# gitouni/Spatial-Temporal-LiDAR-camera-Calibration

Measured on AMD Instinct MI355X. Metric: IBA residual+Jacobian evals/sec, higher is better.
Workload: dtype f64; 1 GPU; configs[1]-shaped synthetic street scene split over the GPUs: 200 keyframes x 10000 pts (2.0M pts), 2000 keypoints/KF, IBACalib cost (3d-2d + 3d-3d plane + hand-eye) + iba_local normal equations per candidate; frames_this_rank=200, points_per_frame=10000, keypoints_per_frame=2000, total_frames=200, total_points=2000000, plane_cache=1, parallelism=frames sharded over 1 GPU(s), 1 all-reduce of 4096 doubles per call, launch=single process, no collective, rccl_ranks=0

## Files before the change

include/iba_mi355x_debug.h:

```cpp
#ifndef IBA_MI355X_DEBUG_H
#define IBA_MI355X_DEBUG_H

#include "iba_mi355x.h"

#ifdef __cplusplus
extern "C" {
#endif

iba_status iba_last_kernel_ms(iba_handle* h, float* frame_kernel_ms, float* total_ms);
iba_status iba_set_timing(iba_handle* h, int32_t enable);
iba_status iba_last_phase_ms(iba_handle* h, float* assoc_kernel_ms, float* nn_kernel_ms, float* rest_ms);
iba_status iba_debug_phase_cycles(iba_handle* h, uint64_t out8[8], int32_t reset);
iba_status iba_debug_phase_cycles12(iba_handle* h, uint64_t out12[12], int32_t reset);
int32_t iba_debug_last_assoc2_threads(const iba_handle* h);
int32_t iba_debug_factor_ranges(const iba_handle* h, int32_t B);
iba_status iba_debug_last_partials(iba_handle* h, double* out, int32_t B);
int32_t iba_debug_last_path(const iba_handle* h);
iba_status iba_debug_plan_groups(const double* x, int32_t B, double max_fx, double max_px, int32_t max_groups, int32_t* group_of, double* group_px, int32_t* n_groups);
int32_t iba_debug_anchor_builds(const iba_handle* h);
int32_t iba_debug_pairs_builds(const iba_handle* h);
int32_t iba_debug_last_pairs_threads(const iba_handle* h);
int32_t iba_debug_pair_list(iba_handle* h, int32_t slot, int32_t frame, uint32_t* out_pairs, int32_t cap);
double iba_debug_nn_left_to_tree(iba_handle* h);
int32_t iba_debug_last_nn_threads(const iba_handle* h);
int32_t iba_debug_last_nn_list(const iba_handle* h);
double iba_debug_mean_pairs(iba_handle* h);
iba_status iba_debug_cand(const double x[7], double out58[58]);
int64_t iba_debug_rescans(iba_handle* h, int32_t reset);
iba_status iba_debug_counters(iba_handle* h, uint32_t out4[4], int32_t reset);
iba_status iba_debug_pair_lists(iba_handle* h, int32_t out3[3]);
iba_status iba_debug_nn(iba_handle* h, int32_t frame, const double* q_xyz, int32_t n, int32_t mode, uint32_t* out_idx, double* out_d2);
iba_status iba_debug_plane(iba_handle* h, int32_t frame, uint32_t point, int32_t which, double out5[5], int32_t* k);
iba_status iba_debug_scan_threads(iba_handle* h, int32_t threads);
int32_t iba_debug_last_scan_threads(const iba_handle* h);

iba_status iba_mads_selftest(int32_t problem, const double* x0, const iba_mads_options* opt, iba_mads_result* res);
iba_status iba_calibrate_mads_trace(iba_handle* h, const double* x0, const iba_mads_options* opt, iba_mads_result* res, double* trace, int32_t cap, int32_t* n_trace);
iba_status iba_calibrate_mads_record(iba_handle* h, const double* x0, const iba_mads_options* opt, iba_mads_result* res, double* trace, int32_t cap, int32_t* n_trace,
                                     int32_t* batch_sizes, int32_t cap_batches, int32_t* n_batches);
// ... 14 lines not shown
```

spatial-temporal-lidar-camera-calibration_amd/__init__.py:

```python
import ctypes as C
import os
import subprocess

import numpy as np

from .abi import (ICP_NMOM, SCAN_NMOM, IbaSubmapDesc, IbaScanEdge, IbaScanOptions, IbaScanResult, IbaIcpOptions, IbaIcpResult, IBA_MAX_BATCH, IbaCreateOptions, IbaLmOptions, IbaLmResult, IbaMadsOptions, IbaMadsResult, IbaBbo, IbaCostOut, IbaNormalOut, IbaParams, IbaProblemDesc, Problem, copy_params,
                  reference_yaml_params)

_HERE = os.path.dirname(os.path.abspath(__file__))
LIB_PATH = os.environ.get("IBA_LIB", os.path.join(_HERE, "libiba_mi355x.so"))
HEADER_PATH = os.path.join(os.path.dirname(_HERE), "include", "iba_mi355x.h")
HEADER_PATHS = [HEADER_PATH, os.path.join(os.path.dirname(_HERE), "include", "iba_mi355x_debug.h")]

STATUS = {0: "IBA_OK", 1: "IBA_ERR_INVALID_ARG", 2: "IBA_ERR_NO_DEVICE", 3: "IBA_ERR_HIP", 4: "IBA_ERR_UNSUPPORTED", 5: "IBA_ERR_STATE", 6: "IBA_ERR_IO"}


class IbaError(RuntimeError):
    def __init__(self, status, msg):
        super().__init__(f"{STATUS.get(status, status)}: {msg}")
        self.status = status


def build_extension(force=False):
    src_dir = os.path.join(_HERE, "csrc")
# ... 403 lines not shown
        self.lib.iba_debug_last_scan_threads.restype = C.c_int32
        return int(self.lib.iba_debug_last_scan_threads(self.h))

    def debug_factor_ranges(self, B):
        self.lib.iba_debug_factor_ranges.argtypes = [C.c_void_p, C.c_int32]
        self.lib.iba_debug_factor_ranges.restype = C.c_int32
        return int(self.lib.iba_debug_factor_ranges(self.h, C.c_int32(B)))

    @property
    def last_nn_threads(self):
        self.lib.iba_debug_last_nn_threads.argtypes = [C.c_void_p]
        self.lib.iba_debug_last_nn_threads.restype = C.c_int32
        return int(self.lib.iba_debug_last_nn_threads(self.h))

    @property
    def last_nn_list(self):
        self.lib.iba_debug_last_nn_list.argtypes = [C.c_void_p]
        self.lib.iba_debug_last_nn_list.restype = C.c_int32
        return int(self.lib.iba_debug_last_nn_list(self.h))

    def debug_last_partials(self, B):
        out = np.zeros((B, partial_stride()))
        self._chk(self.lib.iba_debug_last_partials(self.h, _p(out), C.c_int32(B)))
        return out

    def eval_full_partial(self, x, d_partials_ptr, stream_ptr=None):
        x = self._x(x)
        self._chk(self.lib.iba_eval_full_partial(self.h, _p(x), C.c_int32(len(x)), C.c_void_p(d_partials_ptr), C.c_void_p(stream_ptr)))

    @property
# ... 254 lines not shown
```

spatial-temporal-lidar-camera-calibration_amd/csrc/iba_capi.hip:

```cpp
#include <hip/hip_runtime.h>

#include <algorithm>
#include <atomic>
#include <cfloat>
#include <chrono>
#include <cmath>
#include <cstdio>
#include <cstring>
#include <limits>
#include <string>
#include <thread>
#include <vector>

#include "../../include/iba_mi355x.h"
#include "../../include/iba_mi355x_debug.h"
#include "iba_build.hpp"
#include "iba_host_math.hpp"
#include "iba_internal.hpp"
namespace iba {
const char* debug_env(const char* name) {
    const char* e = std::getenv("IBA_DEBUG_ENV");
    return (e && std::atoi(e) != 0) ? std::getenv(name) : nullptr;
}
}
// ... 58 lines not shown
    int factor_waves_forced = 0;
    F2Layout f2lay{};
    DevBuf<KpRec> d_kp_rec;
    DevBuf<ScanRec> d_scan_rec;
    bool scan_rec_valid = false;
    bool jets_fold = true;
    bool factor_rec = true;
    DevBuf<double> d_ffr;
    DevBuf<double2> d_kp_c;
    int nn_dbg = 0;
    bool nn_list = false;
    int nn_list_workers = 0;
    int n_cus = 256;
    int last_nn_threads = 0;
    int last_nn_list = 0;
    int nn_cg_max = kMaxGroup < 8 ? kMaxGroup : 8;
    int nn_small_min_b = 12;
    bool nn_small = false;
    bool nn_cg_fixed = false;
    bool nn_rounds = true;
    DevBuf<uint32_t> d_lcount, d_lcount_frozen;
    uint32_t max_slots = 0;
    uint32_t lstride = 1;
    int nn_ns = 1;
    DevBuf<double> d_nn_partials;
    hipEvent_t ev_mid = nullptr;
    float last_assoc_ms = 0.f, last_nn_ms = 0.f;
    LdsLayout alay2{};
    int assoc2_flreg_on = 1;
    DevBuf<PairRec> d_pairs;
// ... 203 lines not shown
}

bool layout_nn(const iba_handle* h, NNLayout& L, const int max_group = kMaxGroup) {
    L = NNLayout{};
    uint32_t off = 0;
    L.off_nodes = off; off += 8u * std::max(h->maxNodes, 1u);
    off = align_up(off, 16); L.off_misc = off; off += 128u;
    off = align_up(off, 16); L.off_cd = off; off += 8u * (uint32_t)kCdDoubles * (uint32_t)max_group;
    off = align_up(off, 16); L.off_res = off; off += 8u * kSliceW * (uint32_t)max_group;
    L.off_ovf = off; off += 4u * kSliceW * (uint32_t)max_group;
    L.total = off;
    off = align_up(off, 16); L.off_res2 = off;
    return L.total <= kLdsBytes;
}

int assoc2_q(const iba_handle* h, int threads = kThreads) { return !h->assoc2_flreg_on ? 0 : (h->maxKw <= 2u * (uint32_t)threads ? 2 : (h->maxKw <= 4u * (uint32_t)threads ? 4 : 0)); }
int assoc2_threads(const iba_handle* h, int blocks) {
    if (h->assoc2_threads_forced) return h->assoc2_threads_forced;
    if (blocks < h->assoc2_small_min_blocks) return kThreads;
    return assoc2_q(h, 256) != 0 || assoc2_q(h, kThreads) == 0 ? 256 : kThreads;
}
bool layout_assoc2(const iba_handle* h, LdsLayout& L) {
    const uint32_t rel_slots = std::max<uint32_t>(h->max_slots, 1u);
    const uint32_t red_bytes = 8u * kWaves * 4u + 8u * rel_slots * 12u + 4u * kWaves + 16u;
    L = LdsLayout{};
    L.rel_slots = rel_slots;
    uint32_t off = 0;
    const uint32_t Kp = (std::max(h->maxK, 1u) + 3u) & ~3u;
    L.off_best_d2 = off; off += 8u * Kp;
    L.off_best_idx = off; off += 4u * Kp;
// ... 467 lines not shown
    if (h->timing) HIP_TRY(h, hipEventRecord(h->ev_mid, st));
    if (refit && (want & 1)) {
        if (wide_fit) hipLaunchKernelGGL((iba_fit_kernel<4, 1>), fit_grid, dim3(64), 0, st, dp, h->dprm, fl, h->d_frefit.p, lc, (int)h->lstride, slot_base, want);
        else hipLaunchKernelGGL((iba_fit_kernel<2, 1>), fit_grid, dim3(64), 0, st, dp, h->dprm, fl, h->d_frefit.p, lc, (int)h->lstride, slot_base, want);
        HIP_TRY(h, hipGetLastError());
    }
    bool he_in_search = false;
    if (search) {
        const int he_blocks = (want & 2) ? (B * nf + nn_threads / 2 - 1) / (nn_threads / 2) : 0;
        he_in_search = he_blocks > 0;
        const dim3 grid(8 * per_xcd * ngroups * NS + ((he_blocks + 7) & ~7)), block(nn_threads);
        NNArgs na{dp, h->dprm, nl, (unsigned long long)(h->anchor_set_elems * sizeof(SetPt)), h->nn_rounds ? 1u : 0u, {0}};
        std::memcpy(na.anchor_sel, h->anchor_sel, sizeof(na.anchor_sel));
        const bool wA = (want & 1) != 0, wC = (want & 2) && h->dprm.use_3d3d;
        const SetPt* anchor = sets ? h->d_anchor.p : nullptr;
        auto launch_nn = [&](auto mode_tag) {
            constexpr int MODE = decltype(mode_tag)::value;
            h->last_nn_nrec = nn_nrec; h->last_nn_B = B;
            const int heb = MODE == kRefitSums ? 0 : he_blocks;
            const dim3 grid_m(MODE == kRefitSums ? 8 * per_xcd * ngroups * NS : grid.x);
            auto go = [&](auto kern) { hipLaunchKernelGGL(kern, grid_m, block, nl.total, st, na, dc, B, CG, NS, h->d_nn_partials.p, nn_nrec, fl, lc, (int)h->lstride, h->nn_dbg, h->d_frefit.p, anchor, h->d_he.p, heb); };
            h->last_nn_list = 0; h->last_nn_threads = nn_threads;
            const bool small_bufs = (size_t)B * nf * h->lstride * 16u < 0xFFFFFF00ull && (size_t)kAnchorSets * h->anchor_set_elems * sizeof(SetPt) < 0xFFFFFF00ull && (size_t)dp.n_kp_total * 16u < 0x80000000ull;
            int CGl = 1; { const int capl = B >= 12 ? 8 : (B >= 6 ? 4 : 2); while (CGl < std::min(B, capl)) CGl <<= 1; }
            if (sets && MODE == 0 && h->nn_list && small_bufs && CGl >= 4 && (kSliceW * (uint32_t)CGl) % (2u * (uint32_t)kNLThreads) == 0u && (kSliceW * (uint32_t)CGl) / (uint32_t)kNLThreads <= 4u) {
                NNLayout ll{};
                {
                    uint32_t off = 0;
                    ll.off_nodes = off; off += 8u * std::max(h->maxNodes, 1u);
                    off = align_up(off, 16); ll.off_misc = off; off += 128u;
                    off = align_up(off, 16); ll.off_cd = off; off += 8u * (uint32_t)kCdDoubles * (uint32_t)kNLMaxGroup;
                    off = align_up(off, 16); ll.off_res = off; off += 8u * kSliceW * (uint32_t)kNLMaxGroup;
                    ll.off_ovf = off; off += 4u * kSliceW * (uint32_t)kNLMaxGroup;
                    ll.total = off; off = align_up(off, 16); ll.off_res2 = off;
                }
                const uint32_t lds = align_up(ll.off_res2 + 8u * kSliceW * (uint32_t)kNLMaxGroup, 16);
                const int ngl = (B + CGl - 1) / CGl;
                const int hebl = (want & 2) ? (B * nf + kNLThreads / 2 - 1) / (kNLThreads / 2) : 0;
                const int per_cu = h->nn_list_workers > 0 ? h->nn_list_workers : std::max(1, std::min(4 * IBA_NN_LIST_WAVES * 64 / kNLThreads, (int)(kLdsBytes / lds)));
                const int R = std::max(1, std::min(per_xcd * NS, (h->n_cus * per_cu) / (8 * ngl)));
                h->last_nn_list = R;
                NNArgs nal = na; nal.lay = ll;
                const dim3 grid_l(8 * ngl * R + ((hebl + 7) & ~7));
                auto gol = [&](auto kern) { hipLaunchKernelGGL(kern, grid_l, dim3(kNLThreads), lds, st, nal, dc, B, CGl, NS, R, h->d_nn_partials.p, nn_nrec, fl, lc, (int)h->lstride, h->nn_dbg, anchor, h->d_he.p, hebl); };
                const bool four = (kSliceW * (uint32_t)CGl) / (uint32_t)kNLThreads == 4u;
                if (wA && wC) { if (four) gol(iba_nn_list_kernel<3, 4>); else gol(iba_nn_list_kernel<3, 2>); }
                else if (wA) { if (four) gol(iba_nn_list_kernel<1, 4>); else gol(iba_nn_list_kernel<1, 2>); }
                else { if (four) gol(iba_nn_list_kernel<2, 4>); else gol(iba_nn_list_kernel<2, 2>); }
            }
            else if (MODE == 0 && nn_small) {
                if (sets) { if (wA && wC) go(iba_nn_kernel<3, 0, 1, kNNThreadsSmall>); else if (wA) go(iba_nn_kernel<1, 0, 1, kNNThreadsSmall>); else go(iba_nn_kernel<2, 0, 1, kNNThreadsSmall>); }
                else { if (wA && wC) go(iba_nn_kernel<3, 0, 0, kNNThreadsSmall>); else if (wA) go(iba_nn_kernel<1, 0, 0, kNNThreadsSmall>); else go(iba_nn_kernel<2, 0, 0, kNNThreadsSmall>); }
            }
            else if (sets && MODE != kRefitSums) { if (wA && wC) go(iba_nn_kernel<3, MODE, 1>); else if (wA) go(iba_nn_kernel<1, MODE, 1>); else go(iba_nn_kernel<2, MODE, 1>); }
            else { if (wA && wC) go(iba_nn_kernel<3, MODE, 0>); else if (wA) go(iba_nn_kernel<1, MODE, 0>); else go(iba_nn_kernel<2, MODE, 0>); }
        };
        if (refit) launch_nn(std::integral_constant<int, kRefitSearch>{}); else launch_nn(std::integral_constant<int, 0>{});
        HIP_TRY(h, hipGetLastError());
        if (refit) {
            const int w2 = (wA ? 1 : 0) | (wC ? 2 : 0);
            if (wide_fit) hipLaunchKernelGGL((iba_fit_kernel<4, 2>), fit_grid, dim3(64), 0, st, dp, h->dprm, fl, h->d_frefit.p, lc, (int)h->lstride, slot_base, w2);
            else hipLaunchKernelGGL((iba_fit_kernel<2, 2>), fit_grid, dim3(64), 0, st, dp, h->dprm, fl, h->d_frefit.p, lc, (int)h->lstride, slot_base, w2);
            HIP_TRY(h, hipGetLastError());
// ... 314 lines not shown
    if (const char* e = dbg_env("IBA_ASSOC2_THREADS")) { const int v = std::atoi(e); h->assoc2_threads_forced = (v == 256 || v == kThreads) ? v : 0; }
    if (const char* e = dbg_env("IBA_ASSOC2_SMALL_MIN")) h->assoc2_small_min_blocks = std::max(0, std::atoi(e));
    if (const char* e = dbg_env("IBA_PAIR_GROUPS")) h->max_groups = std::max(1, std::min(kMaxPairGroups, std::atoi(e)));
    if (const char* e = dbg_env("IBA_CHAIN_FOLD")) h->chain_fold = std::atoi(e) != 0;
    if (const char* e = dbg_env("IBA_MAX_CHAIN")) h->chain_cap = std::atoi(e);
    h->chain_cap = std::max(1, std::min(h->chain_cap, (int)kMaxChain));
    if (!layout_assoc(h, h->alay)) { delete h; return fail(nullptr, IBA_ERR_UNSUPPORTED, "keypoints per frame exceed the LDS plan"); }
    if (!layout_assoc2(h, h->alay2) || 8u * (uint32_t)kPairStage + 160u + 2u * std::max(h->maxCoarse, 1u) + 8u * std::max(h->maxK, 1u) > kLdsBytes) h->common_mode = 0;
    if (dbg_env("IBA_LAYOUT_DEBUG")) std::fprintf(stderr, "[iba] assoc LDS: total %u B, queue %u entries, pairs %u, bitmap@%u; maxK %u maxKw %u\n", h->alay.total, h->alay.cand_cap, h->alay.pair_cap, h->alay.off_bitmap, h->maxK, h->maxKw);
    { NNLayout probe; if (!layout_nn(h, probe)) { delete h; return fail(nullptr, IBA_ERR_UNSUPPORTED, "kd tree exceeds the LDS plan of the search kernel"); } }
    h->lstride = std::max(1u, std::min(h->maxK, h->maxKw));
    h->nn_ns = (int)((h->lstride + kSliceW - 1u) / kSliceW) | 1;
    h->nn_small = 8u * std::max(h->maxNodes, 1u) <= 6144u;
    if (const char* e = dbg_env("IBA_NN_SMALL")) h->nn_small = std::atoi(e) != 0;
    if (const char* e = dbg_env("IBA_NN_SMALL_MIN_B")) h->nn_small_min_b = std::max(1, std::atoi(e));

    auto bail = [&](const char* what, hipError_t er) { std::string m = std::string(what) + ": " + hipGetErrorString(er); iba_destroy(h); return fail(nullptr, IBA_ERR_HIP, m); };
#define UP(buf, vec) do { hipError_t _e = h->buf.upload(vec); if (_e != hipSuccess) return bail("upload " #buf, _e); } while (0)
    {
        std::vector<float> frame_box(8 * (size_t)std::max(nf, 1), qnan);
        for (int lf = 0; lf < nf; ++lf) {
            float mn[3] = {INFINITY, INFINITY, INFINITY}, mx[3] = {-INFINITY, -INFINITY, -INFINITY};
            for (uint32_t c0 = 0; c0 < hdr[lf].P; c0 += (uint32_t)kChunk) {
                const float* bx = &chunk_box[8 * (size_t)(hdr[lf].box_base + c0 / (uint32_t)kChunk)];
                for (int a = 0; a < 3; ++a) { if (bx[a] < mn[a]) mn[a] = bx[a]; if (bx[4 + a] > mx[a]) mx[a] = bx[4 + a]; }
            }
            if (hdr[lf].P > 0) for (int a = 0; a < 3; ++a) { frame_box[8 * (size_t)lf + a] = mn[a]; frame_box[8 * (size_t)lf + 4 + a] = mx[a]; }
        }
        h->h_frame_box = frame_box;
        UP(d_frame_box, frame_box);
// ... 94 lines not shown
        const void* a2[12] = {(const void*)iba_assoc2_kernel<2, false, kThreads>, (const void*)iba_assoc2_kernel<2, true, kThreads>, (const void*)iba_assoc2_kernel<4, false, kThreads>, (const void*)iba_assoc2_kernel<4, true, kThreads>,
                              (const void*)iba_assoc2_kernel<0, false, kThreads>, (const void*)iba_assoc2_kernel<0, true, kThreads>,
                              (const void*)iba_assoc2_kernel<2, false, 256>, (const void*)iba_assoc2_kernel<2, true, 256>, (const void*)iba_assoc2_kernel<4, false, 256>, (const void*)iba_assoc2_kernel<4, true, 256>,
                              (const void*)iba_assoc2_kernel<0, false, 256>, (const void*)iba_assoc2_kernel<0, true, 256>};
        for (const void* fn : a2) if (h->common_mode > 0 && (er = hipFuncSetAttribute(fn, hipFuncAttributeMaxDynamicSharedMemorySize, (int)h->alay2.total)) != hipSuccess) return bail("hipFuncSetAttribute", er);
    }
    if ((er = hipFuncSetAttribute((const void*)iba_anchor_kernel, hipFuncAttributeMaxDynamicSharedMemorySize, (int)kLdsBytes)) != hipSuccess) return bail("hipFuncSetAttribute", er);
    const void* nfns[15] = {(const void*)iba_nn_kernel<1, 0, 0>, (const void*)iba_nn_kernel<2, 0, 0>, (const void*)iba_nn_kernel<3, 0, 0>, (const void*)iba_nn_kernel<1, 1, 0>, (const void*)iba_nn_kernel<2, 1, 0>,
                            (const void*)iba_nn_kernel<3, 1, 0>, (const void*)iba_nn_kernel<1, 2, 0>, (const void*)iba_nn_kernel<2, 2, 0>, (const void*)iba_nn_kernel<3, 2, 0>,
                            (const void*)iba_nn_kernel<1, 0, 1>, (const void*)iba_nn_kernel<2, 0, 1>, (const void*)iba_nn_kernel<3, 0, 1>, (const void*)iba_nn_kernel<1, 1, 1>, (const void*)iba_nn_kernel<2, 1, 1>,
                            (const void*)iba_nn_kernel<3, 1, 1>};
    for (const void* fn : nfns)
        if ((er = hipFuncSetAttribute(fn, hipFuncAttributeMaxDynamicSharedMemorySize, (int)kLdsBytes)) != hipSuccess) return bail("hipFuncSetAttribute", er);
    const void* sfns[6] = {(const void*)iba_nn_kernel<1, 0, 0, kNNThreadsSmall>, (const void*)iba_nn_kernel<2, 0, 0, kNNThreadsSmall>, (const void*)iba_nn_kernel<3, 0, 0, kNNThreadsSmall>,
                           (const void*)iba_nn_kernel<1, 0, 1, kNNThreadsSmall>, (const void*)iba_nn_kernel<2, 0, 1, kNNThreadsSmall>, (const void*)iba_nn_kernel<3, 0, 1, kNNThreadsSmall>};
    for (const void* fn : sfns)
        if ((er = hipFuncSetAttribute(fn, hipFuncAttributeMaxDynamicSharedMemorySize, (int)kLdsBytes)) != hipSuccess) return bail("hipFuncSetAttribute", er);
    const void* lfns[6] = {(const void*)iba_nn_list_kernel<1, 2>, (const void*)iba_nn_list_kernel<2, 2>, (const void*)iba_nn_list_kernel<3, 2>, (const void*)iba_nn_list_kernel<1, 4>, (const void*)iba_nn_list_kernel<2, 4>, (const void*)iba_nn_list_kernel<3, 4>};
    for (const void* fn : lfns)
        if ((er = hipFuncSetAttribute(fn, hipFuncAttributeMaxDynamicSharedMemorySize, (int)kLdsBytes)) != hipSuccess) return bail("hipFuncSetAttribute", er);

    {
        DevBuf<int32_t> okb; std::vector<int32_t> z(1, 0);
        er = okb.upload(z);
        if (er != hipSuccess) return bail("kernarg probe", er);
        hipLaunchKernelGGL(iba_kernarg_probe_kernel, dim3(1), dim3(1), 0, h->stream, KArgs{h->dev_problem(), h->dprm, h->alay}, okb.p);
        int32_t okv = 0;
        er = hipStreamSynchronize(h->stream);
        if (er == hipSuccess) er = hipMemcpy(&okv, okb.p, sizeof(okv), hipMemcpyDeviceToHost);
        okb.release();
// ... 209 lines not shown
iba_status iba_debug_phase_cycles(iba_handle* h, uint64_t out8[8], int32_t reset) {
    if (!h || !h->d_diag.p || !out8) return IBA_ERR_INVALID_ARG;
    if (hipSetDevice(h->device) != hipSuccess || hipStreamSynchronize(h->stream) != hipSuccess) return fail(h, IBA_ERR_HIP, "sync");
    if (hipMemcpy(out8, h->d_diag.p + 8, 64, hipMemcpyDeviceToHost) != hipSuccess) return fail(h, IBA_ERR_HIP, "copy");
    if (reset && hipMemset(h->d_diag.p + 8, 0, 64) != hipSuccess) return fail(h, IBA_ERR_HIP, "memset");
    return IBA_OK;
}
iba_status iba_debug_phase_cycles12(iba_handle* h, uint64_t out12[12], int32_t reset) {
    if (!h || !h->d_diag.p || !out12) return IBA_ERR_INVALID_ARG;
    if (hipSetDevice(h->device) != hipSuccess || hipStreamSynchronize(h->stream) != hipSuccess) return fail(h, IBA_ERR_HIP, "sync");
    if (hipMemcpy(out12, h->d_diag.p + 8, 96, hipMemcpyDeviceToHost) != hipSuccess) return fail(h, IBA_ERR_HIP, "copy");
    if (reset && hipMemset(h->d_diag.p + 8, 0, 96) != hipSuccess) return fail(h, IBA_ERR_HIP, "memset");
    return IBA_OK;
}
int32_t iba_debug_last_nn_threads(const iba_handle* h) { return h ? h->last_nn_threads : -1; }
int32_t iba_debug_last_nn_list(const iba_handle* h) { return h ? h->last_nn_list : -1; }
int32_t iba_debug_pairs_builds(const iba_handle* h) { return h ? h->pairs_builds : -1; }
int32_t iba_debug_last_pairs_threads(const iba_handle* h) { return h ? h->last_pairs_threads : -1; }
int32_t iba_debug_pair_list(iba_handle* h, int32_t slot, int32_t frame, uint32_t* out_pairs, int32_t cap) {
    if (h && slot < 0) slot = h->last_mean_pairs_slot;
    if (!h || slot < 0 || slot >= kMaxPairGroups || frame < 0 || frame >= h->n_frames || cap < 0 || (cap > 0 && !out_pairs)) return -1;
    if (!h->d_pairs.p || !h->d_pcounts.p || h->pair_cap <= 0) return 0;
    if (hipSetDevice(h->device) != hipSuccess || hipStreamSynchronize(h->stream) != hipSuccess) return -1;
    uint32_t c = 0;
    if (hipMemcpy(&c, h->d_pcounts.p + h->amap.cnt_off[slot] + (size_t)frame * kCountStride, sizeof(uint32_t), hipMemcpyDeviceToHost) != hipSuccess) return -1;
    const int32_t n = (int32_t)std::min<uint32_t>(c, (uint32_t)h->pair_cap);
    const int32_t m = std::min(n, cap);
    if (m > 0) {
        std::vector<PairRec> v((size_t)m);
        if (hipMemcpy(v.data(), h->d_pairs.p + ((size_t)slot * h->n_frames + (size_t)frame) * (size_t)h->pair_cap, (size_t)m * sizeof(PairRec), hipMemcpyDeviceToHost) != hipSuccess) return -1;
// ... 376 lines not shown
```

spatial-temporal-lidar-camera-calibration_amd/csrc/iba_split_kernels.hpp:

```cpp
#pragma once
#include "iba_kernels.hpp"
#include "iba_pair_plan.hpp"

namespace iba {

#ifndef IBA_PAIRS_CUT
#define IBA_PAIRS_CUT 0
#endif
#ifndef IBA_PAIRS_BLOCK_CUT
#define IBA_PAIRS_BLOCK_CUT 0
#endif
#ifndef IBA_NN_EXP
#define IBA_NN_EXP 0
#endif
#ifndef IBA_NN_THREADS
#define IBA_NN_THREADS 256
#endif
constexpr int kNNThreadsSmall = 64;
constexpr int kNNThreads = IBA_NN_THREADS;
constexpr int kNNWaves = kNNThreads / 64;
#ifndef IBA_NN_SLICE
#define IBA_NN_SLICE 128
#endif
constexpr uint32_t kSliceW = IBA_NN_SLICE;
// ... 5 lines not shown
    uint32_t off_nodes, off_res, off_misc, off_cd, off_ovf, total;
    uint32_t off_res2;
};
constexpr int kCdDoubles = 14;
#ifndef IBA_NN_WAVES
#define IBA_NN_WAVES 5
#endif
#ifndef IBA_NN_ROUND_LEAVES
#define IBA_NN_ROUND_LEAVES 8
#endif
#ifndef IBA_NN_LEAF_BATCH
#define IBA_NN_LEAF_BATCH 4
#endif
#ifndef IBA_NN_SETS_WAVES
#define IBA_NN_SETS_WAVES 4
#endif
constexpr int kAnchorSets = 2;
struct NNArgs {
    DevProblem dp; DevParams prm; NNLayout lay;
    unsigned long long anchor_set_bytes;
    uint32_t nn_rounds;
    uint8_t anchor_sel[kMaxChain];
};

constexpr uint32_t kFlagC = 1u;
constexpr int kRefitSearch = 1, kRefitSums = 2;
#ifdef IBA_DIAG_COUNTERS
#define IBA_DIAG_COUNT(cond, slot) do { if (cond) atomicAdd(dp.diag + (slot), 1u); } while (0)
#else
#define IBA_DIAG_COUNT(cond, slot) do { } while (0)
// ... 1831 lines not shown
                const PlaneRec rc = planes_cost[bp[i]];
                if (!(rc.far_d2 < prm.min_diff_dist2) && !(rc.k < prm.norm_min_pts) && !(rc.reg_sum / (double)(rc.k - 1) > prm.norm_reg_threshold)) { sp.flags |= 2u; sp.nx = rc.nx; sp.ny = rc.ny; sp.nz = rc.nz; }
            }
        }
        *(SetPt*)anchor_pt(row, (uint32_t)i) = sp;
        if (i == 0) hd.d1 = sqrt(bd[0]);
        if (i == 1) hd.da1_lo = sp.da_lo;
        hd.dM = sqrt(bd[i]);
        ++cnt;
    }
    hd.count = cnt;
    if (cnt < (uint32_t)kSetM) hd.dM = INFINITY;
    *(AnchorHdr*)row = hd;
}

template <int WHICH, int REFIT, int SETS, int T = kNNThreads>
__global__ __launch_bounds__(T) __attribute__((amdgpu_waves_per_eu(SETS ? IBA_NN_SETS_WAVES : IBA_NN_WAVES, SETS ? IBA_NN_SETS_WAVES : IBA_NN_WAVES))) void iba_nn_kernel(NNArgs ka_by_value, const Cand* __restrict__ cands, int B, int CG, int NS,
                                                                                                  double* __restrict__ nn_partials, int nn_nrec, uint4* __restrict__ flist,
                                                                                                  const uint32_t* __restrict__ lcount, int flist_stride, int dbg, double4* __restrict__ frefit,
                                                                                                  const SetPt* __restrict__ anchor, double* __restrict__ he_out, int he_blocks) {
    extern __shared__ __align__(16) unsigned char smem[];
    if ((int)blockIdx.x < he_blocks) {
        const int nfh = ka_by_value.dp.n_frames;
        const int i = (int)blockIdx.x * (T / 2) + (int)(threadIdx.x >> 1);
        const bool live = i < B * nfh;
        const int ii = live ? i : 0;
        const double v = he_term(ka_by_value.dp.frames[ii % nfh], cands[ii / nfh], threadIdx.x & 1, live);
        if (live && !(threadIdx.x & 1)) he_out[i] = v;
        return;
    }
    const uint32_t bid = blockIdx.x - (uint32_t)((he_blocks + 7) & ~7);
    constexpr int refit = REFIT;
    typedef __attribute__((address_space(4))) const NNArgs NNArgsC;
    NNArgsC* ka = (NNArgsC*)__builtin_amdgcn_kernarg_segment_ptr();
    (void)ka_by_value;
#define dp (ka->dp)
#define prm (ka->prm)
#define lay (ka->lay)
    constexpr int kMaxGroup = T / 32 < 16 ? T / 32 : 16, kCoopLimit = T / 2;
    static_assert((int)(kSliceW * (uint32_t)kMaxGroup) - kCoopLimit >= T / 2 * 4 && 4 * (2 * kMaxGroup + 4) <= 128, "LDS plan of the block shape");
    const int tid = threadIdx.x, lane = tid & 63;
#ifdef IBA_DIAG_COUNTERS
    unsigned long long nn_t[8] = {0, 0, 0, 0, 0, 0, 0, 0}, nn_last = __builtin_readcyclecounter();
#define NN_TICK(i) do { const unsigned long long _t = __builtin_readcyclecounter(); nn_t[i] += _t - nn_last; nn_last = _t; } while (0)
#else
#define NN_TICK(i) do { } while (0)
#endif
    const int nf = dp.n_frames;
    const int per_xcd = (nf + 7) / 8;
    const int NG = (B + CG - 1) / CG;
    const int per_frame = NG * NS;
    if (blockIdx.x < (uint32_t)((he_blocks + 7) & ~7)) return;
    const int xcd = bid & 7, jj = bid >> 3;
    const int f = xcd + 8 * (jj / per_frame);
    if (f >= nf || jj / per_frame >= per_xcd) return;
    const int g = (jj % per_frame) / NS, sl = (jj % per_frame) % NS;
    const FrameHdr& h = dp.frames[f];
    const uint32_t P = h.P, D = h.depth;
    const int cands_here = min(CG, B - g * CG);
    constexpr uint32_t kWantMask = ((WHICH & 2) ? kFlagC : 0u) | ((WHICH & 1) ? kFlagA : 0u);

    TreeNode* s_nodes = (TreeNode*)(smem + lay.off_nodes);
    double* s_res = (double*)(smem + lay.off_res);
    uint32_t* s_n = (uint32_t*)(smem + lay.off_misc);
    uint32_t* s_ctr = s_n + kMaxGroup;
    double* s_cd = (double*)(smem + lay.off_cd);
    int cg_shift = 0; while ((1 << cg_shift) < CG) ++cg_shift;

    uint32_t my_n = 0u;
    if (tid < cands_here) my_n = lcount[(size_t)(g * CG + tid) * nf + f];
    double my_cd = 0.0;
// ... 109 lines not shown
                    } else {
                        PlaneRec rec; rec.k = 0;
                        if (prm.use_plane) rec = planes_cost[bposC];
                        res = cost_res(prm, prm.use_plane != 0, rec, ex, ey, ez);
                    }
                }
                if (WHICH & 2) s_res[wn - c0] = res;
            };
            uint32_t* s_ovf = (uint32_t*)(smem + lay.off_ovf);
            auto seed = [&](uint32_t wn) {
                const uint2 sd = ((const uint2*)s_res)[wn - c0];
                if ((WHICH & 1) && actA && sd.x != kNone) { const float4 pv = p4[sd.x]; const double dx = ax - (double)pv.x, dy = ay - (double)pv.y, dz = az - (double)pv.z; bestA = (dx * dx + dy * dy) + dz * dz; bposA = sd.x; }
                if ((WHICH & 2) && actC && sd.y != kNone) { const float4 pv = p4[sd.y]; const double dx = qx - (double)pv.x, dy = qy - (double)pv.y, dz = qz - (double)pv.z; bestC = (dx * dx + dy * dy) + dz * dz; bposC = sd.y; }
            };
            uint32_t c_end = c1;
            if (SETS) {
                auto fetch = [&](uint32_t wn, uint4& e, float4& mp) {
                    e = make_uint4(0u, 0u, 0u, 0u); mp = make_float4(0.f, 0.f, 0.f, 0.f);
                    const uint32_t cc = wn & ((1u << cg_shift) - 1u), il = i_lo + (wn >> cg_shift);
                    if (wn < c1 && il < s_n[cc]) { e = flist[entry_at(wn)]; if (e.w & kWantMask) mp = kmp[e.x]; }
                };
                auto pick = [&](uint32_t wn, const uint4& e, const float4& mp, const AnchorHdr& hd, SetPt p0, const unsigned char* row) {
                    bool actA, actC; double ax, ay, az, qx, qy, qz, bestA, bestC; uint32_t bposA, bposC;
                    make_queries_to(wn & ((1u << cg_shift) - 1u), e, mp, actA, actC, ax, ay, az, qx, qy, qz);
                    double S2 = 0.0;
                    if (WHICH & 1) { const double dx = ax - hd.qa[0], dy = ay - hd.qa[1], dz = az - hd.qa[2]; const double dA = (dx * dx + dy * dy) + dz * dz; S2 = actA ? dA : 0.0; }
                    if (WHICH & 2) { const double dx = qx - hd.qa[0], dy = qy - hd.qa[1], dz = qz - hd.qa[2]; const double dC = (dx * dx + dy * dy) + dz * dz; S2 = actC ? fmax(S2, dC) : S2; }
                    auto sqrt_up = [](double v2) -> double { return (double)(__builtin_sqrtf((float)v2) * 1.000001f + 1e-18f); };
                    const double S = sqrt_up(S2);
                    const double radius = (hd.d1 + 2.0 * S) * (1.0 + 1e-12) + 1e-12;
                    const bool quick = radius < hd.dM;
                    auto leave = [&](uint32_t pa, uint32_t pc) { ((uint2*)s_res)[wn - c0] = make_uint2(pa, pc); s_ovf[atomicAdd(&s_ctr[1], 1u)] = wn; };
                    if (hd.count == 0u) { leave(kNone, kNone); return; }
                    bestA = INFINITY; bestC = INFINITY; bposA = kNone; bposC = kNone;
                    uint32_t ia = 0u, ic = 0u;
                    const float rf = quick ? (float)radius * 1.000001f + 1e-30f : INFINITY;
                    {
                        const double x = (double)p0.x, y = (double)p0.y, z = (double)p0.z;
                        if (WHICH & 1) { const double dx = ax - x, dy = ay - y, dz = az - z; nn_merge(bestA, bposA, (dx * dx + dy * dy) + dz * dz, p0.pos, perm_g); }
                        if (WHICH & 2) { const double dx = qx - x, dy = qy - y, dz = qz - z; nn_merge(bestC, bposC, (dx * dx + dy * dy) + dz * dz, p0.pos, perm_g); }
                    }
                    if (hd.count > 1u && hd.da1_lo <= rf) {
                        for (uint32_t si = 1u; si < hd.count; ++si) {
                            const SetPt pv = *anchor_pt(row, si);
                            if (!(pv.da_lo <= rf)) break;
                            const double x = (double)pv.x, y = (double)pv.y, z = (double)pv.z;
                            if ((WHICH & 1) && actA) { const double dx = ax - x, dy = ay - y, dz = az - z; const uint32_t was = bposA; nn_merge(bestA, bposA, (dx * dx + dy * dy) + dz * dz, pv.pos, perm_g); if (bposA != was) ia = si; }
// ... 15 lines not shown
                        if ((WHICH & 2) && actC) {
                            const double ex = (double)pc.x - qx, ey = (double)pc.y - qy, ez = (double)pc.z - qz;
                            if (refit) frefit[at] = make_double4(ex, ey, ez, __longlong_as_double((long long)bposC));
                            else if (pc.flags & 2u) res = fabs(ex * pc.nx + ey * pc.ny + ez * pc.nz);
                            else res = -sqrt((ex * ex + ey * ey) + ez * ez);
                        }
                        if (WHICH & 2) s_res[wn - c0] = res;
                    };
                    if ((ia | ic) == 0u) results(p0.flags, p0);
                    else {
                        const uint32_t fa = ia != 0u ? anchor_pt(row, ia)->flags : p0.flags;
                        const SetPt pc = ic != 0u ? *anchor_pt(row, ic) : p0;
                        results(fa, pc);
                    }
                };
                for (uint32_t wn = (uint32_t)tid; wn < c1; wn += 2u * (uint32_t)T) {
                    uint4 e0, e1; float4 mq0, mq1;
                    fetch(wn, e0, mq0); fetch(wn + (uint32_t)T, e1, mq1);
#ifdef IBA_DIAG_COUNTERS
                    asm volatile("" :: "v"(e0.x), "v"(e1.x), "v"(mq0.x), "v"(mq1.x));
#endif
                    NN_TICK(1);
                    const bool w0 = (e0.w & kWantMask) != 0u, w1 = (e1.w & kWantMask) != 0u;
                    const uint32_t sel0 = s_sel[wn & ((1u << cg_shift) - 1u)], sel1 = s_sel[(wn + (uint32_t)T) & ((1u << cg_shift) - 1u)];
                    const unsigned char* r0 = anchor_row((const unsigned char*)anchor + (size_t)(sel0 != 255u ? sel0 : 0u) * ka->anchor_set_bytes, (size_t)f * dp.max_k + (w0 ? e0.x : 0u));
                    const unsigned char* r1 = anchor_row((const unsigned char*)anchor + (size_t)(sel1 != 255u ? sel1 : 0u) * ka->anchor_set_bytes, (size_t)f * dp.max_k + (w1 ? e1.x : 0u));
                    AnchorHdr h0, h1; SetPt a0, b0;
                    h0.count = h1.count = 0u; h0.dM = h1.dM = -1.0; h0.d1 = h1.d1 = 0.0; h0.da1_lo = h1.da1_lo = INFINITY;
                    a0.flags = b0.flags = 0u;
#if IBA_NN_EXP == 1
                    if (w0 && sel0 != 255u) { h0 = *anchor_hdr(r0); }
                    if (w1 && sel1 != 255u) { h1 = *anchor_hdr(r1); }
#else
                    if (w0 && sel0 != 255u) { h0 = *anchor_hdr(r0); a0 = *anchor_pt(r0, 0u); }
                    if (w1 && sel1 != 255u) { h1 = *anchor_hdr(r1); b0 = *anchor_pt(r1, 0u); }
#endif
#if IBA_NN_EXP == 2
                    asm volatile("" :: "v"(h0.count), "v"(h1.count), "v"(a0.pos), "v"(b0.pos), "v"(h0.dM), "v"(h1.dM), "v"(a0.nz), "v"(b0.nz), "v"(mq0.x), "v"(mq1.x));
                    continue;
#endif
#ifdef IBA_DIAG_COUNTERS
                    asm volatile("" :: "v"(h0.count), "v"(h1.count), "v"(a0.pos), "v"(b0.pos));
#endif
                    NN_TICK(2);
                    if (w0) pick(wn, e0, mq0, h0, a0, r0);
                    if (w1) pick(wn + (uint32_t)T, e1, mq1, h1, b0, r1);
                    NN_TICK(3);
                }
                __syncthreads();
                NN_TICK(4);
                c_end = s_ctr[1];
                left_to_tree = c_end;
                if (tid == 0) *s_ctr = 0u;
                if (c_end != 0u) for (uint32_t i = tid; i < nnodes; i += T) s_nodes[i] = dp.nodes[h.node_base + i];
                __syncthreads();
            }
            const bool coop = SETS && c_end != 0u && c_end <= (uint32_t)kCoopLimit;
            if (coop && dbg != 4) {
                int G = 64; while ((uint32_t)(T / G) < c_end && G > 2) G >>= 1;
                for (uint32_t q = (uint32_t)tid / (uint32_t)G; q < c_end; q += (uint32_t)(T / G)) {
                    const uint32_t wn = s_ovf[q];
                    const uint32_t cc = wn & ((1u << cg_shift) - 1u);
                    const size_t at = entry_at(wn);
                    const uint4 e = flist[at]; const float4 mp = kmp[e.x];
                    make_queries(cc, e, mp);
                    lane_nn_begin(IBA_LANE_NN_PASS);
                    seed(wn);
                    const int round_cap = min(kRoundLeaves, (int)((kSliceW * (uint32_t)kMaxGroup - (uint32_t)kCoopLimit) / (uint32_t)(T / G)));
                    uint32_t* s_leaf = s_ovf + kCoopLimit + ((uint32_t)tid / (uint32_t)G) * (uint32_t)round_cap;
                    if (dbg == 6) {}
                    else if (ka->nn_rounds) do wave_nn_round<WHICH>(IBA_LANE_NN_PASS, tid & (G - 1), G, s_nodes, p4, perm_g, P, D, s_leaf, round_cap); while (go >= 0 && dbg != 7);
                    else do wave_nn_visit<WHICH>(IBA_LANE_NN_PASS, tid & (G - 1), G, s_nodes, p4, perm_g, P, D); while (go >= 0 && dbg != 7);
                    if (dbg != 5) finish(wn, nullptr, nullptr);
                }
            }
            bool exhausted = false;
            if (c_end != 0u && !coop) for (;;) {
                const unsigned long long idle = __ballot(!have);
                if (idle != 0ull && !exhausted) {
                    const uint32_t nidle = (uint32_t)__popcll(idle);
                    uint32_t base = 0u;
                    if (lane == 0) base = atomicAdd(s_ctr, nidle);
                    base = (uint32_t)__builtin_amdgcn_readfirstlane((int)base);
                    exhausted = base + nidle >= c_end;
                    if (!have) {
                        const uint32_t wq = base + (uint32_t)__popcll(idle & ((1ull << lane) - 1ull));
                        const uint32_t wn = SETS ? (wq < c_end ? s_ovf[wq] : c1) : wq;
                        const uint32_t cc = wn & ((1u << cg_shift) - 1u), il = i_lo + (wn >> cg_shift);
                        uint4 e = make_uint4(0u, 0u, 0u, 0u);
                        float4 mp = make_float4(0.f, 0.f, 0.f, 0.f);
                        if (wn < c1 && il < s_n[cc]) { e = flist[entry_at(wn)]; if (e.w & kWantMask) mp = kmp[e.x]; }
                        if (e.w & kWantMask) {
// ... 50 lines not shown
            else if (q == 5 && cc == 0) out = (double)left_to_tree;
            nn_partials[((size_t)(g * CG + cc) * nn_nrec + (size_t)f * NS + sl) * kNNPartial + q] = out;
        }
    }
#ifdef IBA_DIAG_COUNTERS
    NN_TICK(6);
    if (tid == 0 && dp.diag) {
        unsigned long long* d64 = (unsigned long long*)(dp.diag + 8);
        for (int i = 0; i < 7; ++i) atomicAdd(d64 + i, nn_t[i]);
        atomicAdd(d64 + 7, 1ull);
    }
#endif
#undef dp
#undef prm
#undef lay
}


template <int SLOTS, int STAGE>
__global__ __launch_bounds__(64) void iba_fit_kernel(DevProblem dp, DevParams prm, uint4* __restrict__ flist, double4* __restrict__ frefit, const uint32_t* __restrict__ lcount,
                                                     int flist_stride, int slot_base, int want) {
    __shared__ FitLds<SLOTS> s_fit;
    __shared__ uint32_t s_job[64];
    const int nf = dp.n_frames, f = blockIdx.y, b = blockIdx.z, lane = threadIdx.x;
    const uint32_t n = lcount[(size_t)b * nf + f];
    if (blockIdx.x * 64u >= n) return;
    const FrameHdr& h = dp.frames[f];
    const uint32_t i = blockIdx.x * 64u + (uint32_t)lane;
    const size_t at = ((size_t)b * nf + f) * (size_t)flist_stride + i;
    const float4* p4 = dp.pts4 + h.pt_base;
// ... 203 lines not shown
```

Measured before the change: 171,700 evals/s.

## Split NN search into light pick kernel plus redo kernel for unsettled blocks

Adds a two-stage path for the small anchored NN search. A lean pick kernel with a smaller LDS layout and higher waves-per-EU resolves queries from anchor sets only. Any block holding an unsettled query is queued to a device redo list, and a second kernel reruns the full search for just those blocks. The aim is higher occupancy and less tree traversal in the common case, at the cost of an extra launch and recomputing whole blocks that fall back.

```diff
diff --git a/include/iba_mi355x_debug.h b/include/iba_mi355x_debug.h
--- a/include/iba_mi355x_debug.h
+++ b/include/iba_mi355x_debug.h
@@ -23,6 +23,8 @@
 int32_t iba_debug_pair_list(iba_handle* h, int32_t slot, int32_t frame, uint32_t* out_pairs, int32_t cap);
 double iba_debug_nn_left_to_tree(iba_handle* h);
 int32_t iba_debug_last_nn_threads(const iba_handle* h);
+int32_t iba_debug_last_nn_split(const iba_handle* h);
+int32_t iba_debug_nn_redo_count(iba_handle* h);
 int32_t iba_debug_last_nn_list(const iba_handle* h);
 double iba_debug_mean_pairs(iba_handle* h);
 iba_status iba_debug_cand(const double x[7], double out58[58]);
diff --git a/spatial-temporal-lidar-camera-calibration_amd/__init__.py b/spatial-temporal-lidar-camera-calibration_amd/__init__.py
--- a/spatial-temporal-lidar-camera-calibration_amd/__init__.py
+++ b/spatial-temporal-lidar-camera-calibration_amd/__init__.py
@@ -441,6 +441,18 @@
         return int(self.lib.iba_debug_last_nn_threads(self.h))
 
     @property
+    def last_nn_split(self):
+        self.lib.iba_debug_last_nn_split.argtypes = [C.c_void_p]
+        self.lib.iba_debug_last_nn_split.restype = C.c_int32
+        return int(self.lib.iba_debug_last_nn_split(self.h))
+
+    @property
+    def nn_redo_count(self):
+        self.lib.iba_debug_nn_redo_count.argtypes = [C.c_void_p]
+        self.lib.iba_debug_nn_redo_count.restype = C.c_int32
+        return int(self.lib.iba_debug_nn_redo_count(self.h))
+
+    @property
     def last_nn_list(self):
         self.lib.iba_debug_last_nn_list.argtypes = [C.c_void_p]
         self.lib.iba_debug_last_nn_list.restype = C.c_int32
diff --git a/spatial-temporal-lidar-camera-calibration_amd/csrc/iba_capi.hip b/spatial-temporal-lidar-camera-calibration_amd/csrc/iba_capi.hip
--- a/spatial-temporal-lidar-camera-calibration_amd/csrc/iba_capi.hip
+++ b/spatial-temporal-lidar-camera-calibration_amd/csrc/iba_capi.hip
@@ -96,6 +96,12 @@
     int n_cus = 256;
     int last_nn_threads = 0;
     int last_nn_list = 0;
+    bool nn_split = true;
+    bool nn_split_redo_all = false;
+    DevBuf<uint32_t> d_redo;
+    uint32_t redo_cap = 0;
+    unsigned nn_split_seq = 0;
+    int last_nn_split = 0;
     int nn_cg_max = kMaxGroup < 8 ? kMaxGroup : 8;
     int nn_small_min_b = 12;
     bool nn_small = false;
@@ -329,6 +335,16 @@
     return L.total <= kLdsBytes;
 }
 
+void layout_nn_pick(NNLayout& L, const int max_group) {
+    L = NNLayout{};
+    uint32_t off = 0;
+    L.off_nodes = off;
+    L.off_misc = off; off += 128u;
+    off = align_up(off, 16); L.off_cd = off; off += 8u * (uint32_t)kCdDoubles * (uint32_t)max_group;
+    off = align_up(off, 16); L.off_res = off; off += 8u * kSliceW * (uint32_t)max_group;
+    L.off_ovf = off; L.total = off; L.off_res2 = off;
+}
+
 int assoc2_q(const iba_handle* h, int threads = kThreads) { return !h->assoc2_flreg_on ? 0 : (h->maxKw <= 2u * (uint32_t)threads ? 2 : (h->maxKw <= 4u * (uint32_t)threads ? 4 : 0)); }
 int assoc2_threads(const iba_handle* h, int blocks) {
     if (h->assoc2_threads_forced) return h->assoc2_threads_forced;
@@ -826,13 +842,26 @@
         std::memcpy(na.anchor_sel, h->anchor_sel, sizeof(na.anchor_sel));
         const bool wA = (want & 1) != 0, wC = (want & 2) && h->dprm.use_3d3d;
         const SetPt* anchor = sets ? h->d_anchor.p : nullptr;
+        NNLayout pl{};
+        const bool split = nn_small && sets && !refit && h->nn_split && !h->nn_list;
+        if (split) {
+            layout_nn_pick(pl, nn_mg);
+            const uint32_t sblocks = (uint32_t)(8 * per_xcd * ngroups * NS);
+            if (h->redo_cap < sblocks) {
+                HIP_TRY(h, hipStreamSynchronize(st)); HIP_TRY(h, hipStreamSynchronize(h->stream));
+                h->redo_cap = 0; h->d_redo.release();
+                HIP_TRY(h, h->d_redo.alloc((size_t)sblocks + 2));
+                HIP_TRY(h, hipMemset(h->d_redo.p, 0, 2 * sizeof(uint32_t)));
+                h->redo_cap = sblocks;
+            }
+        }
         auto launch_nn = [&](auto mode_tag) {
             constexpr int MODE = decltype(mode_tag)::value;
             h->last_nn_nrec = nn_nrec; h->last_nn_B = B;
             const int heb = MODE == kRefitSums ? 0 : he_blocks;
             const dim3 grid_m(MODE == kRefitSums ? 8 * per_xcd * ngroups * NS : grid.x);
             auto go = [&](auto kern) { hipLaunchKernelGGL(kern, grid_m, block, nl.total, st, na, dc, B, CG, NS, h->d_nn_partials.p, nn_nrec, fl, lc, (int)h->lstride, h->nn_dbg, h->d_frefit.p, anchor, h->d_he.p, heb); };
-            h->last_nn_list = 0; h->last_nn_threads = nn_threads;
+            h->last_nn_list = 0; h->last_nn_threads = nn_threads; h->last_nn_split = 0;
             const bool small_bufs = (size_t)B * nf * h->lstride * 16u < 0xFFFFFF00ull && (size_t)kAnchorSets * h->anchor_set_elems * sizeof(SetPt) < 0xFFFFFF00ull && (size_t)dp.n_kp_total * 16u < 0x80000000ull;
             int CGl = 1; { const int capl = B >= 12 ? 8 : (B >= 6 ? 4 : 2); while (CGl < std::min(B, capl)) CGl <<= 1; }
             if (sets && MODE == 0 && h->nn_list && small_bufs && CGl >= 4 && (kSliceW * (uint32_t)CGl) % (2u * (uint32_t)kNLThreads) == 0u && (kSliceW * (uint32_t)CGl) / (uint32_t)kNLThreads <= 4u) {
@@ -859,6 +888,20 @@
                 if (wA && wC) { if (four) gol(iba_nn_list_kernel<3, 4>); else gol(iba_nn_list_kernel<3, 2>); }
                 else if (wA) { if (four) gol(iba_nn_list_kernel<1, 4>); else gol(iba_nn_list_kernel<1, 2>); }
                 else { if (four) gol(iba_nn_list_kernel<2, 4>); else gol(iba_nn_list_kernel<2, 2>); }
+            }
+            else if (MODE == 0 && split) {
+                const uint32_t sblocks = (uint32_t)(8 * per_xcd * ngroups * NS);
+                uint32_t* const cnt = h->d_redo.p + (h->nn_split_seq & 1u);
+                uint32_t* const other = h->d_redo.p + ((h->nn_split_seq + 1u) & 1u);
+                ++h->nn_split_seq;
+                h->last_nn_split = 1;
+                NNArgs nap = na; nap.lay = pl;
+                const int pdbg = h->nn_split_redo_all ? kNNDbgQueueAll : h->nn_dbg;
+                auto gop = [&](auto kern) { hipLaunchKernelGGL(kern, grid_m, block, pl.total, st, nap, dc, B, CG, NS, h->d_nn_partials.p, nn_nrec, fl, lc, (int)h->lstride, pdbg, anchor, h->d_he.p, heb, cnt, h->d_redo.p + 2, sblocks, other); };
+                auto gor = [&](auto kern) { hipLaunchKernelGGL(kern, dim3(sblocks), block, nl.total, st, na, dc, B, CG, NS, h->d_nn_partials.p, nn_nrec, fl, lc, (int)h->lstride, h->nn_dbg, anchor, cnt, h->d_redo.p + 2, sblocks); };
+                if (wA && wC) { gop(iba_nn_pick_kernel<3>); gor(iba_nn_redo_kernel<3>); }
+                else if (wA) { gop(iba_nn_pick_kernel<1>); gor(iba_nn_redo_kernel<1>); }
+                else { gop(iba_nn_pick_kernel<2>); gor(iba_nn_redo_kernel<2>); }
             }
             else if (MODE == 0 && nn_small) {
                 if (sets) { if (wA && wC) go(iba_nn_kernel<3, 0, 1, kNNThreadsSmall>); else if (wA) go(iba_nn_kernel<1, 0, 1, kNNThreadsSmall>); else go(iba_nn_kernel<2, 0, 1, kNNThreadsSmall>); }
@@ -1203,6 +1246,8 @@
     h->nn_small = 8u * std::max(h->maxNodes, 1u) <= 6144u;
     if (const char* e = dbg_env("IBA_NN_SMALL")) h->nn_small = std::atoi(e) != 0;
     if (const char* e = dbg_env("IBA_NN_SMALL_MIN_B")) h->nn_small_min_b = std::max(1, std::atoi(e));
+    if (const char* e = dbg_env("IBA_NN_SPLIT")) h->nn_split = std::atoi(e) != 0;
+    if (const char* e = dbg_env("IBA_NN_SPLIT_REDO_ALL")) h->nn_split_redo_all = std::atoi(e) != 0;
 
     auto bail = [&](const char* what, hipError_t er) { std::string m = std::string(what) + ": " + hipGetErrorString(er); iba_destroy(h); return fail(nullptr, IBA_ERR_HIP, m); };
 #define UP(buf, vec) do { hipError_t _e = h->buf.upload(vec); if (_e != hipSuccess) return bail("upload " #buf, _e); } while (0)
@@ -1327,6 +1372,9 @@
         if ((er = hipFuncSetAttribute(fn, hipFuncAttributeMaxDynamicSharedMemorySize, (int)kLdsBytes)) != hipSuccess) return bail("hipFuncSetAttribute", er);
     const void* sfns[6] = {(const void*)iba_nn_kernel<1, 0, 0, kNNThreadsSmall>, (const void*)iba_nn_kernel<2, 0, 0, kNNThreadsSmall>, (const void*)iba_nn_kernel<3, 0, 0, kNNThreadsSmall>,
                            (const void*)iba_nn_kernel<1, 0, 1, kNNThreadsSmall>, (const void*)iba_nn_kernel<2, 0, 1, kNNThreadsSmall>, (const void*)iba_nn_kernel<3, 0, 1, kNNThreadsSmall>};
+    const void* rfns[3] = {(const void*)iba_nn_redo_kernel<1>, (const void*)iba_nn_redo_kernel<2>, (const void*)iba_nn_redo_kernel<3>};
+    for (const void* fn : rfns)
+        if ((er = hipFuncSetAttribute(fn, hipFuncAttributeMaxDynamicSharedMemorySize, (int)kLdsBytes)) != hipSuccess) return bail("hipFuncSetAttribute", er);
     for (const void* fn : sfns)
         if ((er = hipFuncSetAttribute(fn, hipFuncAttributeMaxDynamicSharedMemorySize, (int)kLdsBytes)) != hipSuccess) return bail("hipFuncSetAttribute", er);
     const void* lfns[6] = {(const void*)iba_nn_list_kernel<1, 2>, (const void*)iba_nn_list_kernel<2, 2>, (const void*)iba_nn_list_kernel<3, 2>, (const void*)iba_nn_list_kernel<1, 4>, (const void*)iba_nn_list_kernel<2, 4>, (const void*)iba_nn_list_kernel<3, 4>};
@@ -1566,6 +1614,14 @@
     return IBA_OK;
 }
 int32_t iba_debug_last_nn_threads(const iba_handle* h) { return h ? h->last_nn_threads : -1; }
+int32_t iba_debug_last_nn_split(const iba_handle* h) { return h ? h->last_nn_split : -1; }
+int32_t iba_debug_nn_redo_count(iba_handle* h) {
+    if (!h || !h->last_nn_split || !h->d_redo.p) return -1;
+    uint32_t c = 0;
+    if (hipSetDevice(h->device) != hipSuccess || hipStreamSynchronize(h->stream) != hipSuccess) return -1;
+    if (hipMemcpy(&c, h->d_redo.p + ((h->nn_split_seq - 1u) & 1u), sizeof(c), hipMemcpyDeviceToHost) != hipSuccess) return -1;
+    return (int32_t)c;
+}
 int32_t iba_debug_last_nn_list(const iba_handle* h) { return h ? h->last_nn_list : -1; }
 int32_t iba_debug_pairs_builds(const iba_handle* h) { return h ? h->pairs_builds : -1; }
 int32_t iba_debug_last_pairs_threads(const iba_handle* h) { return h ? h->last_pairs_threads : -1; }
diff --git a/spatial-temporal-lidar-camera-calibration_amd/csrc/iba_split_kernels.hpp b/spatial-temporal-lidar-camera-calibration_amd/csrc/iba_split_kernels.hpp
--- a/spatial-temporal-lidar-camera-calibration_amd/csrc/iba_split_kernels.hpp
+++ b/spatial-temporal-lidar-camera-calibration_amd/csrc/iba_split_kernels.hpp
@@ -43,6 +43,12 @@
 #endif
 #ifndef IBA_NN_SETS_WAVES
 #define IBA_NN_SETS_WAVES 4
+#endif
+#ifndef IBA_NN_PICK_STEP
+#define IBA_NN_PICK_STEP 1
+#endif
+#ifndef IBA_NN_PICK_WAVES
+#define IBA_NN_PICK_WAVES 5
 #endif
 constexpr int kAnchorSets = 2;
 struct NNArgs {
@@ -1904,26 +1910,30 @@
     *(AnchorHdr*)row = hd;
 }
 
-template <int WHICH, int REFIT, int SETS, int T = kNNThreads>
-__global__ __launch_bounds__(T) __attribute__((amdgpu_waves_per_eu(SETS ? IBA_NN_SETS_WAVES : IBA_NN_WAVES, SETS ? IBA_NN_SETS_WAVES : IBA_NN_WAVES))) void iba_nn_kernel(NNArgs ka_by_value, const Cand* __restrict__ cands, int B, int CG, int NS,
-                                                                                                  double* __restrict__ nn_partials, int nn_nrec, uint4* __restrict__ flist,
-                                                                                                  const uint32_t* __restrict__ lcount, int flist_stride, int dbg, double4* __restrict__ frefit,
-                                                                                                  const SetPt* __restrict__ anchor, double* __restrict__ he_out, int he_blocks) {
+constexpr int kNNWhole = 0, kNNPick = 1, kNNRedo = 2;
+constexpr int kNNDbgQueueAll = 9;
+template <int WHICH, int REFIT, int SETS, int T, int SPLIT>
+__device__ __forceinline__ void nn_block(const Cand* __restrict__ cands, int B, int CG, int NS,
+                                         double* __restrict__ nn_partials, int nn_nrec, uint4* __restrict__ flist,
+                                         const uint32_t* __restrict__ lcount, int flist_stride, int dbg, double4* __restrict__ frefit,
+                                         const SetPt* __restrict__ anchor, double* __restrict__ he_out, int he_blocks,
+                                         uint32_t* __restrict__ redo_cnt, uint32_t* __restrict__ redo_ids, uint32_t redo_cap, uint32_t* __restrict__ redo_clear) {
+    static_assert(SPLIT == kNNWhole || (SETS == 1 && REFIT == 0 && T == 64), "the split search: anchored lists, memoised planes, one-wave blocks");
     extern __shared__ __align__(16) unsigned char smem[];
-    if ((int)blockIdx.x < he_blocks) {
-        const int nfh = ka_by_value.dp.n_frames;
+    if (SPLIT == kNNRedo && blockIdx.x >= min(*redo_cnt, redo_cap)) return;
+    if (SPLIT != kNNRedo && (int)blockIdx.x < he_blocks) {
+        const int nfh = ((__attribute__((address_space(4))) const NNArgs*)__builtin_amdgcn_kernarg_segment_ptr())->dp.n_frames;
         const int i = (int)blockIdx.x * (T / 2) + (int)(threadIdx.x >> 1);
         const bool live = i < B * nfh;
         const int ii = live ? i : 0;
-        const double v = he_term(ka_by_value.dp.frames[ii % nfh], cands[ii / nfh], threadIdx.x & 1, live);
+        const double v = he_term(((__attribute__((address_space(4))) const NNArgs*)__builtin_amdgcn_kernarg_segment_ptr())->dp.frames[ii % nfh], cands[ii / nfh], threadIdx.x & 1, live);
         if (live && !(threadIdx.x & 1)) he_out[i] = v;
         return;
     }
-    const uint32_t bid = blockIdx.x - (uint32_t)((he_blocks + 7) & ~7);
+    const uint32_t bid = SPLIT == kNNRedo ? redo_ids[blockIdx.x] : blockIdx.x - (uint32_t)((he_blocks + 7) & ~7);
     constexpr int refit = REFIT;
     typedef __attribute__((address_space(4))) const NNArgs NNArgsC;
     NNArgsC* ka = (NNArgsC*)__builtin_amdgcn_kernarg_segment_ptr();
-    (void)ka_by_value;
 #define dp (ka->dp)
 #define prm (ka->prm)
 #define lay (ka->lay)
@@ -1940,11 +1950,16 @@
     const int per_xcd = (nf + 7) / 8;
     const int NG = (B + CG - 1) / CG;
     const int per_frame = NG * NS;
-    if (blockIdx.x < (uint32_t)((he_blocks + 7) & ~7)) return;
+    if (SPLIT != kNNRedo && blockIdx.x < (uint32_t)((he_blocks + 7) & ~7)) return;
     const int xcd = bid & 7, jj = bid >> 3;
     const int f = xcd + 8 * (jj / per_frame);
     if (f >= nf || jj / per_frame >= per_xcd) return;
     const int g = (jj % per_frame) / NS, sl = (jj % per_frame) % NS;
+    auto queue_redo = [&]() { if (tid == 0) { const uint32_t slot = atomicAdd(redo_cnt, 1u); if (slot < redo_cap) redo_ids[slot] = bid; } };
+    if (SPLIT == kNNPick) {
+        if (bid == 0u && tid == 0) *redo_clear = 0u;
+        if (dbg == kNNDbgQueueAll) { queue_redo(); return; }
+    }
     const FrameHdr& h = dp.frames[f];
     const uint32_t P = h.P, D = h.depth;
     const int cands_here = min(CG, B - g * CG);
@@ -2084,6 +2099,7 @@
                 if ((WHICH & 2) && actC && sd.y != kNone) { const float4 pv = p4[sd.y]; const double dx = qx - (double)pv.x, dy = qy - (double)pv.y, dz = qz - (double)pv.z; bestC = (dx * dx + dy * dy) + dz * dz; bposC = sd.y; }
             };
             uint32_t c_end = c1;
+            bool unsettled = false;
             if (SETS) {
                 auto fetch = [&](uint32_t wn, uint4& e, float4& mp) {
                     e = make_uint4(0u, 0u, 0u, 0u); mp = make_float4(0.f, 0.f, 0.f, 0.f);
@@ -2100,7 +2116,10 @@
                     const double S = sqrt_up(S2);
                     const double radius = (hd.d1 + 2.0 * S) * (1.0 + 1e-12) + 1e-12;
                     const bool quick = radius < hd.dM;
-                    auto leave = [&](uint32_t pa, uint32_t pc) { ((uint2*)s_res)[wn - c0] = make_uint2(pa, pc); s_ovf[atomicAdd(&s_ctr[1], 1u)] = wn; };
+                    auto leave = [&](uint32_t pa, uint32_t pc) {
+                        if (SPLIT == kNNPick) unsettled = true;
+                        else { ((uint2*)s_res)[wn - c0] = make_uint2(pa, pc); s_ovf[atomicAdd(&s_ctr[1], 1u)] = wn; }
+                    };
                     if (hd.count == 0u) { leave(kNone, kNone); return; }
                     bestA = INFINITY; bestC = INFINITY; bposA = kNone; bposC = kNone;
                     uint32_t ia = 0u, ic = 0u;
@@ -2146,9 +2165,11 @@
                         results(fa, pc);
                     }
                 };
-                for (uint32_t wn = (uint32_t)tid; wn < c1; wn += 2u * (uint32_t)T) {
+                constexpr bool two = !(SPLIT == kNNPick && IBA_NN_PICK_STEP == 1);
+                for (uint32_t wn = (uint32_t)tid; wn < c1; wn += (two ? 2u : 1u) * (uint32_t)T) {
                     uint4 e0, e1; float4 mq0, mq1;
-                    fetch(wn, e0, mq0); fetch(wn + (uint32_t)T, e1, mq1);
+                    fetch(wn, e0, mq0);
+                    if (two) fetch(wn + (uint32_t)T, e1, mq1); else { e1 = make_uint4(0u, 0u, 0u, 0u); mq1 = make_float4(0.f, 0.f, 0.f, 0.f); }
 #ifdef IBA_DIAG_COUNTERS
                     asm volatile("" :: "v"(e0.x), "v"(e1.x), "v"(mq0.x), "v"(mq1.x));
 #endif
@@ -2179,6 +2200,10 @@
                     if (w1) pick(wn + (uint32_t)T, e1, mq1, h1, b0, r1);
                     NN_TICK(3);
                 }
+                if (SPLIT == kNNPick) {
+                    if (__ballot(unsettled) != 0ull) { queue_redo(); return; }
+                    c_end = 0u;
+                } else {
                 __syncthreads();
                 NN_TICK(4);
                 c_end = s_ctr[1];
@@ -2186,9 +2211,10 @@
                 if (tid == 0) *s_ctr = 0u;
                 if (c_end != 0u) for (uint32_t i = tid; i < nnodes; i += T) s_nodes[i] = dp.nodes[h.node_base + i];
                 __syncthreads();
-            }
-            const bool coop = SETS && c_end != 0u && c_end <= (uint32_t)kCoopLimit;
-            if (coop && dbg != 4) {
+                }
+            }
+            const bool coop = SPLIT != kNNPick && SETS && c_end != 0u && c_end <= (uint32_t)kCoopLimit;
+            if (SPLIT != kNNPick && coop && dbg != 4) {
                 int G = 64; while ((uint32_t)(T / G) < c_end && G > 2) G >>= 1;
                 for (uint32_t q = (uint32_t)tid / (uint32_t)G; q < c_end; q += (uint32_t)(T / G)) {
                     const uint32_t wn = s_ovf[q];
@@ -2207,7 +2233,7 @@
                 }
             }
             bool exhausted = false;
-            if (c_end != 0u && !coop) for (;;) {
+            if (SPLIT != kNNPick && c_end != 0u && !coop) for (;;) {
                 const unsigned long long idle = __ballot(!have);
                 if (idle != 0ull && !exhausted) {
                     const uint32_t nidle = (uint32_t)__popcll(idle);
@@ -2288,6 +2314,32 @@
 #undef dp
 #undef prm
 #undef lay
+}
+
+template <int WHICH, int REFIT, int SETS, int T = kNNThreads>
+__global__ __launch_bounds__(T) __attribute__((amdgpu_waves_per_eu(SETS ? IBA_NN_SETS_WAVES : IBA_NN_WAVES, SETS ? IBA_NN_SETS_WAVES : IBA_NN_WAVES))) void iba_nn_kernel(NNArgs ka_by_value, const Cand* __restrict__ cands, int B, int CG, int NS,
+                                                                                                  double* __restrict__ nn_partials, int nn_nrec, uint4* __restrict__ flist,
+                                                                                                  const uint32_t* __restrict__ lcount, int flist_stride, int dbg, double4* __restrict__ frefit,
+                                                                                                  const SetPt* __restrict__ anchor, double* __restrict__ he_out, int he_blocks) {
+    (void)ka_by_value;
+    nn_block<WHICH, REFIT, SETS, T, kNNWhole>(cands, B, CG, NS, nn_partials, nn_nrec, flist, lcount, flist_stride, dbg, frefit, anchor, he_out, he_blocks, nullptr, nullptr, 0u, nullptr);
+}
+template <int WHICH, int T = kNNThreadsSmall>
+__global__ __launch_bounds__(T) __attribute__((amdgpu_waves_per_eu(IBA_NN_PICK_WAVES, IBA_NN_PICK_WAVES))) void iba_nn_pick_kernel(NNArgs ka_by_value, const Cand* __restrict__ cands, int B, int CG, int NS,
+                                                                                                  double* __restrict__ nn_partials, int nn_nrec, uint4* __restrict__ flist,
+                                                                                                  const uint32_t* __restrict__ lcount, int flist_stride, int dbg,
+                                                                                                  const SetPt* __restrict__ anchor, double* __restrict__ he_out, int he_blocks,
+                                                                                                  uint32_t* __restrict__ redo_cnt, uint32_t* __restrict__ redo_ids, uint32_t redo_cap, uint32_t* __restrict__ redo_clear) {
+    (void)ka_by_value;
+    nn_block<WHICH, 0, 1, T, kNNPick>(cands, B, CG, NS, nn_partials, nn_nrec, flist, lcount, flist_stride, dbg, nullptr, anchor, he_out, he_blocks, redo_cnt, redo_ids, redo_cap, redo_clear);
+}
+template <int WHICH, int T = kNNThreadsSmall>
+__global__ __launch_bounds__(T) __attribute__((amdgpu_waves_per_eu(IBA_NN_SETS_WAVES, IBA_NN_SETS_WAVES))) void iba_nn_redo_kernel(NNArgs ka_by_value, const Cand* __restrict__ cands, int B, int CG, int NS,
+                                                                                                  double* __restrict__ nn_partials, int nn_nrec, uint4* __restrict__ flist,
+                                                                                                  const uint32_t* __restrict__ lcount, int flist_stride, int dbg,
+                                                                                                  const SetPt* __restrict__ anchor, uint32_t* __restrict__ redo_cnt, uint32_t* __restrict__ redo_ids, uint32_t redo_cap) {
+    (void)ka_by_value;
+    nn_block<WHICH, 0, 1, T, kNNRedo>(cands, B, CG, NS, nn_partials, nn_nrec, flist, lcount, flist_stride, dbg, nullptr, anchor, nullptr, 0, redo_cnt, redo_ids, redo_cap, nullptr);
 }
 
 
```

Measured after the change: 155,700 evals/s. 0.907x the previous value.
